# facebookresearch/dmc-net

Measured on AMD Instinct MI355X. Metric: clips/sec (3-seg 224x224) DMC-gen+ResNet-18 train step, higher is better.
Workload: dtype f32

## Files before the change

dmc-net_amd/_lib.py:

```python
import ctypes
import os

PKG = os.path.dirname(os.path.abspath(__file__))
LIB_PATH = os.environ.get("DMC_HIP_LIB", os.path.join(PKG, "libdmcnet_hip.so"))

_P = ctypes.c_void_p
_I = ctypes.c_int
_F = ctypes.c_float
_Z = ctypes.c_size_t
_L = ctypes.c_long

SIGNATURES = {
    "dmc_version": (_I, []),
    "dmc_last_error": (ctypes.c_char_p, []),
    "dmc_profile_mark": (_I, [_P]),
    "dmc_set_option": (_I, [ctypes.c_char_p, _I]),
    "dmc_get_option": (_I, [ctypes.c_char_p]),
    "dmc_gen_tiny_workspace_bytes": (_Z, []),
    "dmc_gen_tiny_saved_bytes": (_Z, [_I, _I, _I]),
    "dmc_gen_tiny_gbuf_bytes": (_Z, [_I, _I, _I]),
    "dmc_gen_tiny_partials_bytes": (_Z, [_I, _I, _I]),
    "dmc_gen_tiny_fwd": (_I, [_P, _P, _P, _P, _P, _P, _P, _I, _I, _I, _I, _P]),
    "dmc_gen_tiny_mse_partials_bytes": (_Z, []),
    "dmc_gen_tiny_fwd_mse": (_I, [_P] * 10 + [_I, _I, _I, _I, _P]),
# ... 29 lines not shown
    "dmc_conv_nhwc_stat_blocks": (_I, [_I] * 8),
    "dmc_conv_nhwc_fwd": (_I, [_P] * 7 + [_I] * 11 + [_P]),
    "dmc_conv_nhwc_stats_final": (_I, [_P, _I, _I, ctypes.c_long, _P, _P, _P, _F, _F, _P]),
    "dmc_conv_nhwc_wt_bytes": (_Z, [_I] * 4),
    "dmc_conv_nhwc_presplit_supported": (_I, [_I, _I]),
    "dmc_conv_nhwc_split": (_I, [_P, _P, _P, _I, _I, _I, _I, _P]),
    "dmc_conv_nhwc_dgrad": (_I, [_P] * 4 + [_I] * 9 + [_P]),
    "dmc_conv_nhwc_dgrad_add": (_I, [_P] * 5 + [_I] * 9 + [_P]),
    "dmc_conv_nhwc_wgrad_bytes": (_Z, [_I] * 9),
    "dmc_conv_nhwc_wgrad": (_I, [_P] * 4 + [_I] * 9 + [_P]),
    "dmc_x3s_slices_bytes": (_Z, [_L, _I]),
    "dmc_x3s_split": (_I, [_P, _P, _L, _I, _P]),
    "dmc_x3s_merge": (_I, [_P, _P, _L, _I, _P]),
    "dmc_x3s_wpack_bytes": (_Z, [_I, _I]),
    "dmc_x3s_pack_weights": (_I, [_P, _P, _P, _I, _I, _P]),
    "dmc_x3s_conv_supported": (_I, [_I] * 5),
    "dmc_x3s_conv_stat_blocks": (_I, [_I] * 4),
    "dmc_x3s_conv_fwd": (_I, [_P] * 4 + [_I] * 6 + [_P]),
    "dmc_x3s_conv_dgrad": (_I, [_P] * 4 + [_I] * 5 + [_P]),
    "dmc_x3s_conv_wgrad_supported": (_I, [_I] * 5),
    "dmc_x3s_conv_wgrad_bytes": (_Z, [_I] * 5),
    "dmc_x3s_conv_wgrad": (_I, [_P] * 4 + [_I] * 5 + [_P]),
    "dmc_x3s_conv_dgrad_s2_supported": (_I, [_I] * 5),
    "dmc_x3s_pack_weights_s2": (_I, [_P, _P, _I, _I, _P]),
    "dmc_x3s_conv_dgrad_s2": (_I, [_P] * 3 + [_I] * 5 + [_P]),
    "dmc_x3q_wpack_bytes": (_Z, [_I, _I]),
    "dmc_x3q_supported": (_I, [_I] * 5),
    "dmc_x3q_stat_blocks": (_I, [_I] * 4),
    "dmc_x3q_split": (_I, [_P, _P, _I, _I, _I, _I, _P]),
    "dmc_x3q_merge": (_I, [_P, _P, _I, _I, _I, _I, _P]),
# ... 107 lines not shown
```

dmc-net_amd/csrc/conv_x3s.hip:

```cpp
#include "dmc_common.h"
#include "x3s_common.h"
#include <type_traits>

using namespace dmc;
using namespace dmc::x3;

namespace {

__global__ __launch_bounds__(256) void x3s_split_kernel(const float* __restrict__ x, unsigned short* __restrict__ xs, long M, int C) {
    const int c8 = C >> 3;
    const long total = M * c8;
    const int nchunk = C >> 4;
    for (long o = (long)blockIdx.x * 256 + threadIdx.x; o < total; o += (long)gridDim.x * 256) {
        const long m = o / c8;
        const int g = (int)(o - m * c8);
        const float4 a = reinterpret_cast<const float4*>(x)[2 * o], b = reinterpret_cast<const float4*>(x)[2 * o + 1];
        const float v[8] = {a.x, a.y, a.z, a.w, b.x, b.y, b.z, b.w};
        x3s_store8(xs, v, (size_t)M, nchunk, (size_t)m, g);
    }
}

__global__ __launch_bounds__(256) void x3s_merge_kernel(const unsigned short* __restrict__ xs, float* __restrict__ x, long M, int C) {
    const long total = M * C;
    const size_t plane = (size_t)M * 16;
    const int nchunk = C >> 4;
    for (long o = (long)blockIdx.x * 256 + threadIdx.x; o < total; o += (long)gridDim.x * 256) {
        const long m = o / C;
        const int c = (int)(o - m * C);
        const size_t w = ((size_t)(c >> 4) * M + m) * 16 + (c & 15);
        const float a = __uint_as_float((unsigned)xs[w] << 16);
        const float b = __uint_as_float((unsigned)xs[(size_t)nchunk * plane + w] << 16);
        const float d = __uint_as_float((unsigned)xs[(size_t)2 * nchunk * plane + w] << 16);
        x[o] = (a + b) + d;
    }
}

__global__ __launch_bounds__(256) void x3s_pack_w_kernel(const float* __restrict__ w, unsigned short* __restrict__ wf,
                                                         unsigned short* __restrict__ wt, int Cout, int Cin, int mirror) {
    const bool transposed = blockIdx.y == 1;
    unsigned short* dst = transposed ? wt : wf;
    if (!dst) return;
    const int R = transposed ? Cin : Cout, K = transposed ? Cout : Cin;
    const int nchunk = K >> 4;
    const long total = (long)R * 9 * K;
    for (long i = (long)blockIdx.x * 256 + threadIdx.x; i < total; i += (long)gridDim.x * 256) {
        long t = i;
        const int kk = (int)(t & 15); t >>= 4;
        const int rl = (int)(t & 63); t >>= 6;
        const int tap = (int)(t % 9); t /= 9;
        const int ch = (int)(t % nchunk);
        const int rt = (int)(t / nchunk);
        const int r = rt * 64 + rl, k = ch * 16 + kk;
        const float v = transposed ? w[((long)k * 9 + (mirror ? 8 - tap : tap)) * Cin + r] : w[((long)r * 9 + tap) * Cin + k];
        unsigned u0, u1, u2;
        split3(v, u0, u1, u2);
        const size_t base = ((((size_t)(rt * nchunk + ch) * 9 + tap) * 3) * 64 + rl) * 16 + (kk ^ (((rl >> 3) & 1) << 3));
        dst[base] = (unsigned short)(u0 >> 16);
        dst[base + 64 * 16] = (unsigned short)(u1 >> 16);
        dst[base + 2 * 64 * 16] = (unsigned short)(u2 >> 16);
    }
}

struct X3Args {
    const void* xs;
    const void* wp;
    float* y;
    const float* addend;
    double* stat_part;
    int N, H, W, K, R;
    int M;
    unsigned plane_bytes;
    const float* bnb_y = nullptr;
    const float* bnb_stats = nullptr;
    const float* bnb_gamma = nullptr;
    const float* bnb_beta = nullptr;
    const unsigned char* bnb_mask = nullptr;
    int bnb_relu = 0;
    double* bnb_part = nullptr;
    int part_blocks = -1;
    int ablate;
};

template <int WM, int WN, int TM, int TN, int PPMAX, bool STAG = false, int CLS = 1>
__global__ __launch_bounds__(WM * WN * 64) void x3s_conv_kernel(X3Args a) {
    constexpr int NW = WM * WN, BM = 32 * TM * WM, BN = 32 * TN * WN;
    static_assert(BN == 64, "packed weight image is 64 rows wide");
    static_assert(PPMAX % 32 == 0 || PPMAX % 32 == 1, "patch transfers move 32 pixel rows");
    constexpr int PSL = PPMAX * 32;
    constexpr int PB = 3 * PSL;
    constexpr int WB = 3 * 3 * BN * 32;
    constexpr int WOFF = 2 * PB;
    static_assert(!STAG || NW >= 4, "two transfer groups need four waves");
    constexpr int NA = STAG ? NW / 2 : NW, NB = NW - (STAG ? NA : 0);
    constexpr int NDW = (PPMAX / 32 + NA - 1) / NA;
    constexpr int NEW = WB / 1024;
    constexpr int NEWW = (NEW + NB - 1) / NB;
    extern __shared__ __attribute__((aligned(1024))) char lds_x3[];

    const int tid = threadIdx.x, lane = tid & 63;
    const int wave = __builtin_amdgcn_readfirstlane(tid >> 6);
    const int wm = wave % WM, wn = wave / WM;
// ... 2 lines not shown

    const int HW = a.H * a.W, PW = a.W;
    constexpr int ZROW = PPMAX - 1;
    const int m0 = blockIdx.x * BM;
    const int mlast = (m0 + BM < a.M ? m0 + BM : a.M) - 1;
    const int r_first = m0 / PW, r_last = mlast / PW;
    const int f0 = (r_first > 0 ? r_first - 1 : 0) * PW;
    const int f1 = (r_last + 2) * PW < a.M ? (r_last + 2) * PW : a.M;
    const int PP = f1 - f0;
    const int ND = (PP + 31) >> 5;

    unsigned pvoff[NDW];
#pragma unroll
    for (int k = 0; k < NDW; ++k) {
        const int pr = 32 * (wave + NA * k) + (lane >> 1), h = lane & 1;
        pvoff[k] = pr < PP ? (unsigned)(f0 + pr) * 32u + (unsigned)((h ^ ((pr >> 3) & 1)) << 4) : OOB;
    }
    int xaddr[TM][9];
#pragma unroll
    for (int i = 0; i < TM; ++i) {
        int m = m0 + (wm * TM + i) * 32 + l31;
        if (m > mlast) m = mlast;
        const int n = m / HW, rem = m - n * HW, yy = rem / a.W, xx = rem - yy * a.W;
        const int pp = m - f0;
#pragma unroll
        for (int t = 0; t < 9; ++t) {
            const int dx = CLS == 4 ? (t % 3 == 0 ? 1 : 0) : t % 3 - 1, dy = CLS == 4 ? (t / 3 == 0 ? 1 : 0) : t / 3 - 1;
            const int row = (xx + dx >= 0 && xx + dx < a.W && yy + dy >= 0 && yy + dy < a.H) ? pp + dy * PW + dx : ZROW;
            xaddr[i][t] = row * 32 + ((khalf ^ ((row >> 3) & 1)) << 4);
        }
    }
    const int waddr = (wn * TN * 32 + l31) * 32 + ((khalf ^ ((l31 >> 3) & 1)) << 4);

    const u32x4 srd_x = make_srd(a.xs);
    const int nchunk = a.K >> 4, S = 3 * nchunk;
    const u32x4 srd_w = make_srd(reinterpret_cast<const char*>(a.wp) + (size_t)blockIdx.y * S * WB);
    const unsigned lane16 = (unsigned)lane * 16u;

    const bool grp_a = wave < NA, grp_b = !STAG || wave >= NA;
    const int wb = STAG ? wave - NA : wave;
    auto dma_weight = [&](int step, int wbuf, int k) {
        const int e = wb + NB * k;
        if (e < NEW) dma_buf16(srd_w, lane16, (unsigned)(step * WB + e * 1024), lds0 + WOFF + wbuf * WB + e * 1024);
    };
    auto dma_patch = [&](int chunk, int slice, int pbuf, int k) {
        const int d = wave + NA * k;
        if (d < ND) dma_buf16(srd_x, pvoff[k], (unsigned)(slice * nchunk + chunk) * a.plane_bytes, lds0 + pbuf * PB + slice * PSL + d * 1024);
// ... 103 lines not shown
                if (s + 2 < S) issue_weights(s + 2, wbuf);
                if (vc < nchunk) issue_patch(vc, q == 2 ? 0 : q + 1, q == 2 ? pbuf : (pbuf ^ 1));
            }
            if (s + 1 < S) load_frags(NP{}, NWB{}, NT{}, FB);
            mfma_frags(FA, T2{}, nothing);
        }
    };
    using I0 = std::integral_constant<int, 0>;
    using I1 = std::integral_constant<int, 1>;
    using Q0 = std::integral_constant<int, 0>;
    using Q1 = std::integral_constant<int, 1>;
    using Q2 = std::integral_constant<int, 2>;

    if (tid < 12)
        *reinterpret_cast<float4*>(lds_x3 + (tid >> 1) * PSL + ZROW * 32 + (tid & 1) * 16) = make_float4(0.f, 0.f, 0.f, 0.f);
    issue_weights(0, 0);
    issue_patch(0, 0, 0); issue_patch(0, 1, 0); issue_patch(0, 2, 0);
    asm volatile("s_waitcnt vmcnt(0)" ::: "memory");
    __builtin_amdgcn_s_barrier();
    if (dma_on) {
        if (!STAG && S > 1) issue_weights(1, 1);
        if (nchunk > 1) issue_patch(1, 0, 1);
    }
    Frag F0, F1;
    load_frags(I0{}, I0{}, Q0{}, F0);
#pragma unroll 1
    for (int c = 0; c < ((DMC_ABL(a.ablate) & 256) ? 0 : nchunk); c += 2) {
        step(I0{}, I0{}, Q0{}, F0, F1, c);
        step(I0{}, I1{}, Q1{}, F1, F0, c);
        step(I0{}, I0{}, Q2{}, F0, F1, c);
        step(I1{}, I1{}, Q0{}, F1, F0, c + 1);
        step(I1{}, I0{}, Q1{}, F0, F1, c + 1);
        step(I1{}, I1{}, Q2{}, F1, F0, c + 1);
    }

    static_assert(WN == 1 && TN == 2, "epilogue: a wave owns all 64 channels of its pixels");
    constexpr int EP = 272, ETILE = 32 * TM * EP;
    char* etile = lds_x3 + wave * ETILE;
    const int mw0 = m0 + wm * TM * 32;
    const int rbase = blockIdx.y * BN;
#pragma unroll
    for (int cl = 0; cl < CLS; ++cl) {
#pragma unroll
        for (int i = 0; i < TM; ++i) {
            const bool ok = mw0 + 32 * i + l31 <= mlast;
#pragma unroll
            for (int j = 0; j < TN; ++j)
#pragma unroll
                for (int g = 0; g < 4; ++g) {
                    float4 v = make_float4(acc[cl][i][j][4 * g], acc[cl][i][j][4 * g + 1], acc[cl][i][j][4 * g + 2], acc[cl][i][j][4 * g + 3]);
                    if (!ok) v = make_float4(0.f, 0.f, 0.f, 0.f);
                    *reinterpret_cast<float4*>(etile + (32 * i + l31) * EP + (32 * j + 8 * g + 4 * khalf) * 4) = v;
                }
        }
        if (!(DMC_ABL(a.ablate) & 128)) {
#pragma unroll
            for (int it = 0; it < 8 * TM; ++it) {
                const int prow = 4 * it + (lane >> 4);
                const int m = mw0 + prow;
// ... 86 lines not shown
    int worst = 0;
    long tiles = (M + BM - 1) / BM;
    if (tiles > W) tiles = W;
    for (long t = 0; t < tiles; ++t) {
        const long m0 = t * BM, ml = (m0 + BM < M ? m0 + BM : M) - 1;
        const long r0 = m0 / W, r1 = ml / W;
        const long f0 = (r0 > 0 ? r0 - 1 : 0) * W, f1 = (r1 + 2) * W;
        if ((int)(f1 - f0) + 1 > worst) worst = (int)(f1 - f0) + 1;
    }
    return worst;
}

struct X3Cfg { int id, BM, PPMAX, threads; };
constexpr X3Cfg X3CFGS[] = {{0, 256, 608, 512}, {1, 128, 320, 256}, {2, 64, 192, 128}, {3, 256, 608, 256}, {4, 128, 225, 256}};

bool x3s_shape_ok(int N, int H, int W, int K, int R) {
    if (N <= 0 || H <= 0 || W <= 0 || K % 32 != 0 || R % 64 != 0 || K <= 0 || R <= 0) return false;
    const long M = (long)N * H * W;
    return M * (K > R ? K : R) * 6 < (1L << 31);
}

int x3s_choose(int N, int H, int W, int R) {
    const long M = (long)N * H * W;
    const int forced = option(OPT_CONV_CFG);
    if (forced >= 101 && forced <= 105 && patch_pixels_max(N, H, W, X3CFGS[forced - 101].BM) <= X3CFGS[forced - 101].PPMAX) return forced - 101;
    if (forced != 106 && patch_pixels_max(N, H, W, X3CFGS[4].BM) <= X3CFGS[4].PPMAX && ((M + X3CFGS[4].BM - 1) / X3CFGS[4].BM) * (R / 64) >= 512)
        return 4;
    int fallback = -1;
    for (const X3Cfg& c : X3CFGS) {
        if (c.id > 2 || patch_pixels_max(N, H, W, c.BM) > c.PPMAX) continue;
        const long wgs = ((M + c.BM - 1) / c.BM) * (R / 64);
        if (wgs >= 160) return c.id;
        fallback = c.id;
    }
    return fallback;
}

template <int WM, int TM, int PPMAX>
int launch_x3s(const X3Args& a, hipStream_t s) {
    constexpr int BM = 32 * TM * WM;
    constexpr size_t op_bytes = 2 * 3 * PPMAX * 32 + 2 * 3 * 3 * 64 * 32, ep_bytes = 2 * (size_t)BM * 272 + 8192;
    constexpr size_t lds_bytes = op_bytes > ep_bytes ? op_bytes : ep_bytes;
    dim3 grid((a.M + BM - 1) / BM, a.R / 64);
    if ((a.stat_part || a.bnb_part) && a.part_blocks >= 0 && (unsigned)a.part_blocks != grid.x)
        return fail(DMC_E_INVALID, "x3s_conv: statistics partials have %d rows but this launch writes %u (dmc_x3s_conv_stat_blocks was "
                                   "called under another conv_cfg option?)", a.part_blocks, grid.x);
    if constexpr (WM >= 4) {
        if (!(option(OPT_CONV_ABLATE) & 512)) {
            static LdsLimit lim_attr2;
    const hipError_t attr2 = lim_attr2.raise(reinterpret_cast<const void*>(&x3s_conv_kernel<WM, 1, TM, 2, PPMAX, true>), (int)lds_bytes);
            if (attr2 != hipSuccess) return fail(DMC_E_LAUNCH, "x3s_conv: cannot raise the dynamic LDS limit: %s", hipGetErrorString(attr2));
            x3s_conv_kernel<WM, 1, TM, 2, PPMAX, true><<<grid, WM * 64, lds_bytes, s>>>(a);
            return check_launch("x3s_conv");
        }
    }
    static LdsLimit lim_attr;
    const hipError_t attr = lim_attr.raise(reinterpret_cast<const void*>(&x3s_conv_kernel<WM, 1, TM, 2, PPMAX>), (int)lds_bytes);
    if (attr != hipSuccess) return fail(DMC_E_LAUNCH, "x3s_conv: cannot raise the dynamic LDS limit: %s", hipGetErrorString(attr));
    x3s_conv_kernel<WM, 1, TM, 2, PPMAX><<<grid, WM * 64, lds_bytes, s>>>(a);
    return check_launch("x3s_conv");
}

struct X3Bnb { const float *y, *stats, *gamma, *beta; const unsigned char* mask; int relu; double* part; };

int run_x3s(const void* xs, const void* wp, const float* addend, float* y, double* stat_part, int part_blocks, int N, int H, int W,
            int K, int R, hipStream_t s, const X3Bnb* bnb = nullptr) {
    if (!xs || !wp || !y) return fail(DMC_E_INVALID, "x3s_conv: null pointer");
    if (!x3s_shape_ok(N, H, W, K, R)) return fail(DMC_E_INVALID, "x3s_conv: unsupported shape N=%d H=%d W=%d K=%d R=%d", N, H, W, K, R);
    const int cfg = x3s_choose(N, H, W, R);
    X3Args a;
    a.xs = xs; a.wp = wp; a.y = y; a.addend = addend; a.stat_part = stat_part;
    a.N = N; a.H = H; a.W = W; a.K = K; a.R = R; a.M = N * H * W;
    a.plane_bytes = (unsigned)a.M * 32u;
    a.part_blocks = part_blocks;
    if ((stat_part || bnb) && part_blocks <= 0) return fail(DMC_E_INVALID, "x3s_conv: stat_blocks must be the row count of the partials");
    if (bnb) {
        a.bnb_y = bnb->y; a.bnb_stats = bnb->stats; a.bnb_gamma = bnb->gamma; a.bnb_beta = bnb->beta; a.bnb_mask = bnb->mask;
        a.bnb_relu = bnb->relu; a.bnb_part = bnb->part;
    }
    a.ablate = option(OPT_CONV_ABLATE);
    if (DMC_ABL(a.ablate) & 32) a.stat_part = nullptr;
    switch (cfg) {
        case 0: return launch_x3s<8, 1, 608>(a, s);
        case 1: return launch_x3s<4, 1, 320>(a, s);
        case 2: return launch_x3s<2, 1, 192>(a, s);
        case 3: return launch_x3s<4, 2, 608>(a, s);
        case 4: return launch_x3s<4, 1, 225>(a, s);
        default: return fail(DMC_E_INVALID, "x3s_conv: the patch of a %d x %d image does not fit the LDS", H, W);
    }
}

struct X3WgArgs {
    const void* xs;
    const void* dys;
    float* part;
    int N, H, Cin, Cout;
    unsigned plane_bytes;
    int steps, per_group, tiles_ci;
};

template <int W_, int R>
struct WgGeom {
// ... 227 lines not shown

int dmc_x3s_split(const float* x, void* xs, long M, int C, dmc_stream_t stream) {
    if (!x || !xs || M <= 0 || C <= 0 || C % 16 != 0) return fail(DMC_E_INVALID, "dmc_x3s_split: bad argument");
    x3s_split_kernel<<<stream_blocks(M * (C / 8)), 256, 0, (hipStream_t)stream>>>(x, static_cast<unsigned short*>(xs), M, C);
    return check_launch("x3s_split");
}

int dmc_x3s_merge(const void* xs, float* x, long M, int C, dmc_stream_t stream) {
    if (!x || !xs || M <= 0 || C <= 0 || C % 16 != 0) return fail(DMC_E_INVALID, "dmc_x3s_merge: bad argument");
    x3s_merge_kernel<<<stream_blocks(M * C), 256, 0, (hipStream_t)stream>>>(static_cast<const unsigned short*>(xs), x, M, C);
    return check_launch("x3s_merge");
}

size_t dmc_x3s_wpack_bytes(int Cin, int Cout) { return (size_t)Cin * (size_t)Cout * 9 * 6; }

int dmc_x3s_pack_weights(const float* w, void* wpack_f, void* wpack_t, int Cin, int Cout, dmc_stream_t stream) {
    if (!w || (!wpack_f && !wpack_t) || Cin % 64 != 0 || Cout % 64 != 0 || Cin <= 0 || Cout <= 0)
        return fail(DMC_E_INVALID, "dmc_x3s_pack_weights: bad argument");
    const long total = (long)Cin * Cout * 9;
    x3s_pack_w_kernel<<<dim3(stream_blocks(total) > 1024 ? 1024 : stream_blocks(total), 2), 256, 0, (hipStream_t)stream>>>(
        w, static_cast<unsigned short*>(wpack_f), static_cast<unsigned short*>(wpack_t), Cout, Cin, 1);
    return check_launch("x3s_pack_w");
}

int dmc_x3s_conv_supported(int N, int H, int W, int Cin, int Cout) {
    return Cin % 64 == 0 && Cout % 64 == 0 && x3s_shape_ok(N, H, W, Cin, Cout) && x3s_shape_ok(N, H, W, Cout, Cin) &&
           x3s_choose(N, H, W, Cout) >= 0 && x3s_choose(N, H, W, Cin) >= 0 ? 1 : 0;
}

int dmc_x3s_conv_stat_blocks(int N, int H, int W, int Cout) {
    const int cfg = x3s_choose(N, H, W, Cout);
    if (cfg < 0) return 0;
    const long M = (long)N * H * W;
    return (int)((M + X3CFGS[cfg].BM - 1) / X3CFGS[cfg].BM);
}

// ... 37 lines not shown
        case 14: return launch_x3s_wgrad<14, 4>(p, a, dw, s);
        default: return launch_x3s_wgrad<7, 9>(p, a, dw, s);
    }
}

int dmc_x3s_conv_dgrad_s2_supported(int N, int OH, int OW, int Cin, int Cout) {
    return Cin % 64 == 0 && Cout % 64 == 0 && x3s_shape_ok(N, OH, OW, Cout, Cin) && (long)N * OH * OW * 4 * Cin * 4 < (1L << 40) &&
           patch_pixels_max(N, OH, OW, 128) <= 320 ? 1 : 0;
}

int dmc_x3s_pack_weights_s2(const float* w, void* wpack_t2, int Cin, int Cout, dmc_stream_t stream) {
    if (!w || !wpack_t2 || Cin % 64 != 0 || Cout % 64 != 0 || Cin <= 0 || Cout <= 0)
        return fail(DMC_E_INVALID, "dmc_x3s_pack_weights_s2: bad argument");
    const long total = (long)Cin * Cout * 9;
    x3s_pack_w_kernel<<<dim3(stream_blocks(total) > 1024 ? 1024 : stream_blocks(total), 2), 256, 0, (hipStream_t)stream>>>(
        w, nullptr, static_cast<unsigned short*>(wpack_t2), Cout, Cin, 0);
    return check_launch("x3s_pack_w_s2");
}

int dmc_x3s_conv_dgrad_s2(const void* dys, const void* wpack_t2, float* dx, int N, int OH, int OW, int Cin, int Cout,
                          dmc_stream_t stream) {
    if (!dys || !wpack_t2 || !dx) return fail(DMC_E_INVALID, "dmc_x3s_conv_dgrad_s2: null pointer");
    if (!dmc_x3s_conv_dgrad_s2_supported(N, OH, OW, Cin, Cout))
        return fail(DMC_E_INVALID, "dmc_x3s_conv_dgrad_s2: unsupported shape N=%d OH=%d OW=%d Cin=%d Cout=%d", N, OH, OW, Cin, Cout);
    X3Args a;
    a.xs = dys; a.wp = wpack_t2; a.y = dx; a.addend = nullptr; a.stat_part = nullptr;
    a.N = N; a.H = OH; a.W = OW; a.K = Cout; a.R = Cin; a.M = N * OH * OW;
    a.plane_bytes = (unsigned)a.M * 32u;
    a.ablate = option(OPT_CONV_ABLATE);
    constexpr size_t lds_bytes = 2 * 3 * 320 * 32 + 2 * 3 * 3 * 64 * 32;
    static LdsLimit lim_attr;
    const hipError_t attr = lim_attr.raise(reinterpret_cast<const void*>(&x3s_conv_kernel<4, 1, 1, 2, 320, true, 4>), (int)lds_bytes);
    if (attr != hipSuccess) return fail(DMC_E_LAUNCH, "x3s_conv_dgrad_s2: cannot raise the dynamic LDS limit: %s", hipGetErrorString(attr));
    dim3 grid((a.M + 127) / 128, Cin / 64);
    x3s_conv_kernel<4, 1, 1, 2, 320, true, 4><<<grid, 256, lds_bytes, (hipStream_t)stream>>>(a);
    return check_launch("x3s_conv_dgrad_s2");
}

int dmc_x3s_conv_dgrad_bnb(const void* dys, const void* wpack_t, const float* addend, float* dx, const float* bn_y,
// ... 14 lines not shown
```

dmc-net_amd/csrc/dmc_common.h:

```cpp
#pragma once
#include <hip/hip_runtime.h>
#include <stdarg.h>
#include <stdio.h>

#include <atomic>

#include "dmcnet_hip.h"

namespace dmc {

inline char* err_buf() {
    static thread_local char buf[512] = {0};
    return buf;
}
inline int fail(int code, const char* fmt, ...) {
    va_list ap;
    va_start(ap, fmt);
    vsnprintf(err_buf(), 512, fmt, ap);
    va_end(ap);
    return code;
}
inline int check_launch(const char* what) {
    hipError_t e = hipGetLastError();
    if (e != hipSuccess) return fail(DMC_E_LAUNCH, "%s: %s", what, hipGetErrorString(e));
// ... 2 lines not shown

struct LdsLimit {
    std::atomic<unsigned long long> raised{0};
    hipError_t raise(const void* kernel, int bytes) {
        int dev = 0;
        hipError_t e = hipGetDevice(&dev);
        if (e != hipSuccess) return e;
        if (dev >= 0 && dev < 64 && ((raised.load(std::memory_order_relaxed) >> dev) & 1ull)) return hipSuccess;
        e = hipFuncSetAttribute(kernel, hipFuncAttributeMaxDynamicSharedMemorySize, bytes);
        if (e == hipSuccess && dev >= 0 && dev < 64) raised.fetch_or(1ull << dev, std::memory_order_relaxed);
        return e;
    }
};

enum Option { OPT_GEN_LAYER_PATH = 0, OPT_GEN_GATHER, OPT_GEN_FUSE45, OPT_GEN_WGRAD_PATH, OPT_GEN_FUSE_FWD,
              OPT_GEN_FUSE_BWD, OPT_GEN_FRAMES, OPT_CONV_PATH, OPT_CONV_CFG, OPT_CONV_ABLATE, OPT_GEN_ABLATE, OPT_CONV_ARITH, OPT_CONV3D_WGRAD, OPT_GEN_X3, OPT_GEN_WINO, OPT_GEN_STAGGER, OPT_GEN_FUSED, OPT_GRID_RESERVE_CUS, OPT_COUNT };
int option(Option o);
inline int persistent_cus(int hw) {
    const int r = option(OPT_GRID_RESERVE_CUS);
    int n = hw - (r > 0 ? r : 0);
    n -= n % 8;
    return n < 8 ? (hw < 8 ? hw : 8) : n;
}
#ifdef DMC_MEASURE
#define DMC_ABL(x) (x)
constexpr bool MEASURE_BUILD = true;
#else
#define DMC_ABL(x) 0
constexpr bool MEASURE_BUILD = false;
#endif
constexpr bool measure_only(int o) { return o == OPT_GEN_ABLATE || o == OPT_CONV_ABLATE || o == OPT_GEN_STAGGER; }
// ... 130 lines not shown
```

dmc-net_amd/csrc/losses.hip:

```cpp
#include <atomic>
#include <string.h>

#include "dmc_common.h"

using namespace dmc;

namespace {

constexpr int MSE_BLOCKS = 2048;

__device__ __forceinline__ double wave_sum(double v) {
#pragma unroll
    for (int o = 32; o > 0; o >>= 1) v += __shfl_down(v, o, 64);
    return v;
}
__device__ __forceinline__ float wave_sum(float v) {
#pragma unroll
    for (int o = 32; o > 0; o >>= 1) v += __shfl_down(v, o, 64);
    return v;
}
__device__ __forceinline__ float wave_max(float v) {
#pragma unroll
    for (int o = 32; o > 0; o >>= 1) v = fmaxf(v, __shfl_down(v, o, 64));
    return v;
// ... 96 lines not shown
                const float g = t_ok ? (p - (c == t ? 1.f : 0.f)) * inv_n : NAN;
                for (int s = 0; s < S; ++s) grad[((size_t)b * S + s) * C + c] = g;
            }
        }
    }
    if (lane == 0) wave_loss[wave] = loss;
    __syncthreads();
    if (threadIdx.x == 0) {
        float s = 0.f;
        for (int w = 0; w < 16; ++w) s += wave_loss[w];
        *loss_out = s / (float)B;
    }
}

const char* const OPTION_NAMES[OPT_COUNT] = {"gen_layer_path", "gen_gather", "gen_fuse45", "gen_wgrad_path",
                                             "gen_fuse_fwd", "gen_fuse_bwd", "gen_frames", "conv_path", "conv_cfg", "conv_ablate", "gen_ablate", "conv_arith", "conv3d_wgrad", "gen_x3", "gen_wino", "gen_stagger", "gen_fused", "grid_reserve_cus"};
std::atomic<int> g_options[OPT_COUNT] = {{1}, {1}, {1}, {5}, {1}, {1}, {0}, {1}, {0}, {0}, {0}, {1}, {2}, {2}, {768}, {0}, {1}, {0}};
int option_index(const char* name) {
    if (!name) return -1;
    for (int i = 0; i < OPT_COUNT; ++i)
        if (strcmp(name, OPTION_NAMES[i]) == 0) return i;
    return -1;
}

}

namespace dmc {
int option(Option o) { return !MEASURE_BUILD && measure_only(o) ? 0 : g_options[o].load(std::memory_order_relaxed); }
}

__global__ void dmc_profile_mark_kernel() {}

// ... 68 lines not shown
```

dmc-net_amd/csrc/x3s_common.h:

```cpp
#pragma once
#include "dmc_common.h"

namespace dmc {
namespace x3 {

typedef float f32x16 __attribute__((ext_vector_type(16)));
typedef __bf16 bf16x8 __attribute__((ext_vector_type(8)));
typedef unsigned u32x4 __attribute__((ext_vector_type(4)));
typedef const __attribute__((address_space(3))) char* lds_cptr;

__device__ __forceinline__ f32x16 mfma_bf16(const u32x4& a, const u32x4& b, const f32x16& c) {
    return __builtin_amdgcn_mfma_f32_32x32x16_bf16(__builtin_bit_cast(bf16x8, a), __builtin_bit_cast(bf16x8, b), c, 0, 0, 0);
}

__device__ __forceinline__ void split3(float v, unsigned& u0, unsigned& u1, unsigned& u2) {
    u0 = __float_as_uint(v);
    const float r1 = v - __uint_as_float(u0 & 0xffff0000u);
    u1 = __float_as_uint(r1);
    u2 = __float_as_uint(r1 - __uint_as_float(u1 & 0xffff0000u));
}
__device__ __forceinline__ unsigned pack_hi(unsigned hi_of_second, unsigned hi_of_first) {
    return __builtin_amdgcn_perm(hi_of_second, hi_of_first, 0x07060302u);
}

// ... 45 lines not shown
__device__ __forceinline__ void wg_group_base(const WgGroupPos& p, int N, int W, unsigned img_bytes, unsigned& tbase, unsigned& img_off) {
    const bool in = p.n >= 0 && p.n < N;
    tbase = in ? (unsigned)((p.y - 1) * W) * 32u : NOPIX;
    img_off = in ? (unsigned)p.n * img_bytes : 0u;
}
__device__ __forceinline__ unsigned wg_lane_off(unsigned tbase, unsigned pre, unsigned img_bytes) {
    const unsigned t = tbase + pre;
    return t < img_bytes ? t : OOB;
}

typedef float f32x4 __attribute__((ext_vector_type(4)));
__device__ __forceinline__ f32x4 mfma16(const u32x4& a, const u32x4& b, const f32x4& c) {
    return __builtin_amdgcn_mfma_f32_16x16x32_bf16(__builtin_bit_cast(bf16x8, a), __builtin_bit_cast(bf16x8, b), c, 0, 0, 0);
}

__device__ __forceinline__ void split8(const float4& lo, const float4& hi, u32x4& s0, u32x4& s1, u32x4& s2) {
    const float v[8] = {lo.x, lo.y, lo.z, lo.w, hi.x, hi.y, hi.z, hi.w};
    unsigned u0[8], u1[8], u2[8];
#pragma unroll
    for (int e = 0; e < 8; ++e) split3(v[e], u0[e], u1[e], u2[e]);
#pragma unroll
    for (int e = 0; e < 4; ++e) {
        s0[e] = pack_hi(u0[2 * e + 1], u0[2 * e]);
        s1[e] = pack_hi(u1[2 * e + 1], u1[2 * e]);
        s2[e] = pack_hi(u2[2 * e + 1], u2[2 * e]);
    }
}

}
}
// ... 1 lines not shown
```

include/dmcnet_hip.h:

```cpp
#ifndef DMCNET_HIP_H
#define DMCNET_HIP_H

#include <stddef.h>
#include <stdint.h>

#ifdef __cplusplus
extern "C" {
#endif

#define DMC_OK 0
#define DMC_E_INVALID (-1)
#define DMC_E_LAUNCH (-2)

typedef void* dmc_stream_t;

int dmc_version(void);
const char* dmc_last_error(void);
int dmc_set_option(const char* name, int value);
int dmc_get_option(const char* name);
int dmc_profile_mark(dmc_stream_t stream);


size_t dmc_gen_tiny_workspace_bytes(void);
size_t dmc_gen_tiny_saved_bytes(int N, int H, int W);
// ... 94 lines not shown
size_t dmc_conv_nhwc_wt_bytes(int Cin, int Cout, int KH, int KW);
int dmc_conv_nhwc_presplit_supported(int Cin, int Cout);
int dmc_conv_nhwc_split(const float* w, void* wpack_f, void* wpack_t, int Cin, int Cout, int KH, int KW, dmc_stream_t stream);
int dmc_conv_nhwc_dgrad(const float* dy, const float* w, float* wt, float* dx, int N, int H, int W, int Cin,
                        int Cout, int KH, int KW, int stride, int pad, dmc_stream_t stream);
int dmc_conv_nhwc_dgrad_add(const float* dy, const float* w, float* wt, const float* addend, float* dx, int N, int H, int W,
                            int Cin, int Cout, int KH, int KW, int stride, int pad, dmc_stream_t stream);
size_t dmc_conv_nhwc_wgrad_bytes(int N, int H, int W, int Cin, int Cout, int KH, int KW, int stride, int pad);
int dmc_conv_nhwc_wgrad(const float* x, const float* dy, float* dw, float* workspace, int N, int H, int W,
                        int Cin, int Cout, int KH, int KW, int stride, int pad, dmc_stream_t stream);

size_t dmc_x3s_slices_bytes(long M, int C);
int dmc_x3s_split(const float* x, void* xs, long M, int C, dmc_stream_t stream);
int dmc_x3s_merge(const void* xs, float* x, long M, int C, dmc_stream_t stream);
size_t dmc_x3s_wpack_bytes(int Cin, int Cout);
int dmc_x3s_pack_weights(const float* w, void* wpack_f, void* wpack_t, int Cin, int Cout, dmc_stream_t stream);
int dmc_x3s_conv_supported(int N, int H, int W, int Cin, int Cout);
int dmc_x3s_conv_stat_blocks(int N, int H, int W, int Cout);
int dmc_x3s_conv_fwd(const void* xs, const void* wpack_f, float* y, double* stat_partials, int stat_blocks, int N, int H, int W,
                     int Cin, int Cout, dmc_stream_t stream);
int dmc_x3s_conv_dgrad(const void* dys, const void* wpack_t, const float* addend, float* dx, int N, int H, int W, int Cin,
                       int Cout, dmc_stream_t stream);
int dmc_x3s_conv_wgrad_supported(int N, int H, int W, int Cin, int Cout);
size_t dmc_x3s_conv_wgrad_bytes(int N, int H, int W, int Cin, int Cout);
int dmc_x3s_conv_wgrad(const void* xs, const void* dys, float* dw, float* workspace, int N, int H, int W, int Cin, int Cout,
                       dmc_stream_t stream);
int dmc_x3s_conv_dgrad_s2_supported(int N, int OH, int OW, int Cin, int Cout);
int dmc_x3s_pack_weights_s2(const float* w, void* wpack_t2, int Cin, int Cout, dmc_stream_t stream);
int dmc_x3s_conv_dgrad_s2(const void* dys, const void* wpack_t2, float* dx, int N, int OH, int OW, int Cin, int Cout,
                          dmc_stream_t stream);
// ... 151 lines not shown
```

Baseline: 3578.

## Add 16x16x32 MFMA inner loop and matching weight layout for x3s convolutions

Adds an alternative inner loop to the split-bf16 3x3 convolution kernel that uses 16x16x32 bf16 MFMA instead of 32x32x16. It regroups the K dimension into 9 groups of tap/chunk pairs per 32 channels, with a new packed weight layout, a three-buffer weight pipeline and a staged epilogue. By default it is enabled for 64x64 and 512x512 channel shapes. The aim is higher matrix-core throughput and fewer LDS loads per MFMA. In exchange it adds a host-side registry that checks the packed layout matches the loop chosen at launch, plus extra register pressure.

```diff
diff --git a/dmc-net_amd/_lib.py b/dmc-net_amd/_lib.py
--- a/dmc-net_amd/_lib.py
+++ b/dmc-net_amd/_lib.py
@@ -67,6 +67,9 @@
     "dmc_x3s_merge": (_I, [_P, _P, _L, _I, _P]),
     "dmc_x3s_wpack_bytes": (_Z, [_I, _I]),
     "dmc_x3s_pack_weights": (_I, [_P, _P, _P, _I, _I, _P]),
+    "dmc_x3s_conv_loop": (_I, [_I] * 3),
+    "dmc_x3s_kgroup_unit": (_I, [_I] * 2),
+    "dmc_x3s_wpack_indices": (_I, [_I] * 3 + [_P]),
     "dmc_x3s_conv_supported": (_I, [_I] * 5),
     "dmc_x3s_conv_stat_blocks": (_I, [_I] * 4),
     "dmc_x3s_conv_fwd": (_I, [_P] * 4 + [_I] * 6 + [_P]),
diff --git a/dmc-net_amd/csrc/conv_x3s.hip b/dmc-net_amd/csrc/conv_x3s.hip
--- a/dmc-net_amd/csrc/conv_x3s.hip
+++ b/dmc-net_amd/csrc/conv_x3s.hip
@@ -1,6 +1,8 @@
 #include "dmc_common.h"
 #include "x3s_common.h"
+#include <mutex>
 #include <type_traits>
+#include <unordered_map>
 
 using namespace dmc;
 using namespace dmc::x3;
@@ -36,10 +38,12 @@
 }
 
 __global__ __launch_bounds__(256) void x3s_pack_w_kernel(const float* __restrict__ w, unsigned short* __restrict__ wf,
-                                                         unsigned short* __restrict__ wt, int Cout, int Cin, int mirror) {
+                                                         unsigned short* __restrict__ wt, int Cout, int Cin, int mirror, int loop_f,
+                                                         int loop_t) {
     const bool transposed = blockIdx.y == 1;
     unsigned short* dst = transposed ? wt : wf;
     if (!dst) return;
+    const bool loop16 = (transposed ? loop_t : loop_f) != 0;
     const int R = transposed ? Cin : Cout, K = transposed ? Cout : Cin;
     const int nchunk = K >> 4;
     const long total = (long)R * 9 * K;
@@ -54,10 +58,15 @@
         const float v = transposed ? w[((long)k * 9 + (mirror ? 8 - tap : tap)) * Cin + r] : w[((long)r * 9 + tap) * Cin + k];
         unsigned u0, u1, u2;
         split3(v, u0, u1, u2);
-        const size_t base = ((((size_t)(rt * nchunk + ch) * 9 + tap) * 3) * 64 + rl) * 16 + (kk ^ (((rl >> 3) & 1) << 3));
-        dst[base] = (unsigned short)(u0 >> 16);
-        dst[base + 64 * 16] = (unsigned short)(u1 >> 16);
-        dst[base + 2 * 64 * 16] = (unsigned short)(u2 >> 16);
+        if (loop16) {
+            dst[x3s_w16_index(K, r, k, tap, 0)] = (unsigned short)(u0 >> 16);
+            dst[x3s_w16_index(K, r, k, tap, 1)] = (unsigned short)(u1 >> 16);
+            dst[x3s_w16_index(K, r, k, tap, 2)] = (unsigned short)(u2 >> 16);
+        } else {
+            dst[x3s_w32_index(K, r, k, tap, 0)] = (unsigned short)(u0 >> 16);
+            dst[x3s_w32_index(K, r, k, tap, 1)] = (unsigned short)(u1 >> 16);
+            dst[x3s_w32_index(K, r, k, tap, 2)] = (unsigned short)(u2 >> 16);
+        }
     }
 }
 
@@ -81,10 +90,11 @@
     int ablate;
 };
 
-template <int WM, int WN, int TM, int TN, int PPMAX, bool STAG = false, int CLS = 1>
+template <int WM, int WN, int TM, int TN, int PPMAX, bool STAG = false, int CLS = 1, int MF = 0>
 __global__ __launch_bounds__(WM * WN * 64) void x3s_conv_kernel(X3Args a) {
     constexpr int NW = WM * WN, BM = 32 * TM * WM, BN = 32 * TN * WN;
     static_assert(BN == 64, "packed weight image is 64 rows wide");
+    static_assert(!MF || (TM == 1 && CLS == 1), "the 16x16x32 loop is built for one 32-pixel tile per wave, stride 1");
     static_assert(PPMAX % 32 == 0 || PPMAX % 32 == 1, "patch transfers move 32 pixel rows");
     constexpr int PSL = PPMAX * 32;
     constexpr int PB = 3 * PSL;
@@ -117,7 +127,7 @@
 #pragma unroll
     for (int k = 0; k < NDW; ++k) {
         const int pr = 32 * (wave + NA * k) + (lane >> 1), h = lane & 1;
-        pvoff[k] = pr < PP ? (unsigned)(f0 + pr) * 32u + (unsigned)((h ^ ((pr >> 3) & 1)) << 4) : OOB;
+        pvoff[k] = pr < PP ? (unsigned)(f0 + pr) * 32u + (unsigned)((h ^ (MF ? 0 : (pr >> 3) & 1)) << 4) : OOB;
     }
     int xaddr[TM][9];
 #pragma unroll
@@ -134,6 +144,27 @@
         }
     }
     const int waddr = (wn * TN * 32 + l31) * 32 + ((khalf ^ ((l31 >> 3) & 1)) << 4);
+    const int l15 = lane & 15, sel = lane >> 5, h16 = ((lane >> 4) & 1) << 4;
+    int xg[2][X3S_G16];
+    if constexpr (MF) {
+#pragma unroll
+        for (int i = 0; i < 2; ++i) {
+            int m = m0 + wm * 32 + 16 * i + l15;
+            if (m > mlast) m = mlast;
+            const int n = m / HW, rem = m - n * HW, yy = rem / a.W, xx = rem - yy * a.W;
+            const int pp = m - f0;
+            int rowt[9];
+#pragma unroll
+            for (int t = 0; t < 9; ++t) {
+                const int dx = t % 3 - 1, dy = t / 3 - 1;
+                rowt[t] = (xx + dx >= 0 && xx + dx < a.W && yy + dy >= 0 && yy + dy < a.H) ? pp + dy * PW + dx : ZROW;
+            }
+#pragma unroll
+            for (int g = 0; g < X3S_G16; ++g)
+                xg[i][g] = (sel ? rowt[x3s_g16_tap(g, 1)] * 32 + x3s_g16_chunk(g, 1) * PB : rowt[x3s_g16_tap(g, 0)] * 32 + x3s_g16_chunk(g, 0) * PB) + h16;
+        }
+    }
+    const int waddr16 = sel * 512 + l15 * 32 + h16;
 
     const u32x4 srd_x = make_srd(a.xs);
     const int nchunk = a.K >> 4, S = 3 * nchunk;
@@ -267,24 +298,159 @@
 
     if (tid < 12)
         *reinterpret_cast<float4*>(lds_x3 + (tid >> 1) * PSL + ZROW * 32 + (tid & 1) * 16) = make_float4(0.f, 0.f, 0.f, 0.f);
-    issue_weights(0, 0);
-    issue_patch(0, 0, 0); issue_patch(0, 1, 0); issue_patch(0, 2, 0);
-    asm volatile("s_waitcnt vmcnt(0)" ::: "memory");
-    __builtin_amdgcn_s_barrier();
-    if (dma_on) {
-        if (!STAG && S > 1) issue_weights(1, 1);
-        if (nchunk > 1) issue_patch(1, 0, 1);
-    }
-    Frag F0, F1;
-    load_frags(I0{}, I0{}, Q0{}, F0);
+    if constexpr (MF) {
+        constexpr int WG = 3 * BN * 64;
+        static_assert(3 * WG == 2 * WB, "three group buffers take the place of the two tap-row buffers");
+        constexpr int NEW16 = WG / 1024, NEWW16 = (NEW16 + NB - 1) / NB;
+        const int NG = (nchunk >> 1) * X3S_G16;
+        auto dma_weight16 = [&](int G, int wbuf, int k) {
+            const int e = wb + NB * k;
+            if (e < NEW16) dma_buf16(srd_w, lane16, (unsigned)(G * WG + e * 1024), lds0 + WOFF + wbuf * WG + e * 1024);
+        };
+        f32x4 acc16[2][4];
+#pragma unroll
+        for (int i = 0; i < 2; ++i)
+#pragma unroll
+            for (int j = 0; j < 4; ++j)
+#pragma unroll
+                for (int e = 0; e < 4; ++e) acc16[i][j][e] = 0.f;
+        struct Frag16 { u32x4 X[2][3], W[4][3]; };
+        auto load_frag16 = [&](auto gic, auto wbufc, auto qc, Frag16& f) {
+            constexpr int gi = decltype(gic)::value, wbuf = decltype(wbufc)::value, q = decltype(qc)::value, sl = q / 6, o = q % 6;
+            if constexpr (o < 4)
+                f.W[o][sl] = *reinterpret_cast<const __attribute__((address_space(3))) u32x4*>(L + waddr16 + (WOFF + wbuf * WG + (sl * 4 + o) * 1024));
+            else
+                f.X[o - 4][sl] = *reinterpret_cast<const __attribute__((address_space(3))) u32x4*>(L + xg[o - 4][gi] + sl * PSL);
+        };
+        auto group16 = [&](auto gic, Frag16& FA, Frag16& FB, int c) {
+            constexpr int gi = decltype(gic)::value;
+            using GN = std::integral_constant<int, (gi + 1) % X3S_G16>;
+            using WN_ = std::integral_constant<int, (gi + 1) % 3>;
+            constexpr int wfill = (gi + 2) % 3;
+            constexpr int pslice = gi == 0 ? 1 : gi == 1 ? 2 : gi == 4 ? 0 : gi == 5 ? 1 : gi == 6 ? 2 : gi == 8 ? 0 : -1;
+            constexpr int pdc = gi <= 1 ? 1 : gi == 8 ? 3 : 2, pbuf = gi >= 4 && gi <= 6 ? 0 : 1;
+            const int G = (c >> 1) * X3S_G16 + gi;
+            if (DMC_ABL(a.ablate) & 16) asm volatile("s_waitcnt lgkmcnt(0)" ::: "memory");
+            else asm volatile("s_waitcnt vmcnt(0) lgkmcnt(0)" ::: "memory");
+            __builtin_amdgcn_s_barrier();
+            const bool gow = grp_b && dma_on && G + 2 < NG;
+            const bool gop = pslice >= 0 && grp_a && dma_on && c + pdc < nchunk;
+            if constexpr (!STAG) {
+                if (gow) {
+#pragma unroll
+                    for (int k = 0; k < NEWW16; ++k) dma_weight16(G + 2, wfill, k);
+                }
+                if (gop) {
+#pragma unroll
+                    for (int k = 0; k < NDW; ++k) dma_patch(c + pdc, pslice < 0 ? 0 : pslice, pbuf, k);
+                }
+            }
+            auto product = [&](auto pc) {
+                constexpr int p = decltype(pc)::value;
+                constexpr int WS[6] = {0, 0, 0, 1, 1, 2}, XS[6] = {2, 1, 0, 1, 0, 0};
+                load_frag16(GN{}, WN_{}, std::integral_constant<int, 3 * p>{}, FB);
+                load_frag16(GN{}, WN_{}, std::integral_constant<int, 3 * p + 1>{}, FB);
+                load_frag16(GN{}, WN_{}, std::integral_constant<int, 3 * p + 2>{}, FB);
+#pragma unroll
+                for (int i = 0; i < 2; ++i)
+#pragma unroll
+                    for (int j = 0; j < 4; ++j) acc16[i][j] = mfma16(FA.W[j][WS[p]], FA.X[i][XS[p]], acc16[i][j]);
+#pragma unroll
+                for (int k = 0; k < 3; ++k) {
+                    __builtin_amdgcn_sched_group_barrier(0x008, 1, 0);
+                    __builtin_amdgcn_sched_group_barrier(0x100, 1, 0);
+                }
+                __builtin_amdgcn_sched_group_barrier(0x008, 5, 0);
+                if constexpr (STAG) {
+                    if (gow) {
+#pragma unroll
+                        for (int k = p; k < NEWW16; k += 6) dma_weight16(G + 2, wfill, k);
+                    }
+                    if (gop) {
+#pragma unroll
+                        for (int k = p; k < NDW; k += 6) dma_patch(c + pdc, pslice < 0 ? 0 : pslice, pbuf, k);
+                    }
+                }
+            };
+            product(std::integral_constant<int, 0>{}); product(std::integral_constant<int, 1>{});
+            product(std::integral_constant<int, 2>{}); product(std::integral_constant<int, 3>{});
+            product(std::integral_constant<int, 4>{}); product(std::integral_constant<int, 5>{});
+        };
+        auto pair16 = [&](Frag16& FA, Frag16& FB, int c) {
+            group16(std::integral_constant<int, 0>{}, FA, FB, c); group16(std::integral_constant<int, 1>{}, FB, FA, c);
+            group16(std::integral_constant<int, 2>{}, FA, FB, c); group16(std::integral_constant<int, 3>{}, FB, FA, c);
+            group16(std::integral_constant<int, 4>{}, FA, FB, c); group16(std::integral_constant<int, 5>{}, FB, FA, c);
+            group16(std::integral_constant<int, 6>{}, FA, FB, c); group16(std::integral_constant<int, 7>{}, FB, FA, c);
+            group16(std::integral_constant<int, 8>{}, FA, FB, c);
+        };
+        if (grp_b) {
+#pragma unroll
+            for (int k = 0; k < NEWW16; ++k) dma_weight16(0, 0, k);
+        }
+        issue_patch(0, 0, 0); issue_patch(0, 1, 0); issue_patch(0, 2, 0);
+        asm volatile("s_waitcnt vmcnt(0)" ::: "memory");
+        __builtin_amdgcn_s_barrier();
+        if (dma_on) {
+            if (grp_b && NG > 1) {
+#pragma unroll
+                for (int k = 0; k < NEWW16; ++k) dma_weight16(1, 1, k);
+            }
+            if (nchunk > 1) issue_patch(1, 0, 1);
+        }
+        Frag16 F0, F1;
+        {
+            using Z = std::integral_constant<int, 0>;
+            load_frag16(Z{}, Z{}, std::integral_constant<int, 0>{}, F0); load_frag16(Z{}, Z{}, std::integral_constant<int, 1>{}, F0);
+            load_frag16(Z{}, Z{}, std::integral_constant<int, 2>{}, F0); load_frag16(Z{}, Z{}, std::integral_constant<int, 3>{}, F0);
+            load_frag16(Z{}, Z{}, std::integral_constant<int, 4>{}, F0); load_frag16(Z{}, Z{}, std::integral_constant<int, 5>{}, F0);
+            load_frag16(Z{}, Z{}, std::integral_constant<int, 6>{}, F0); load_frag16(Z{}, Z{}, std::integral_constant<int, 7>{}, F0);
+            load_frag16(Z{}, Z{}, std::integral_constant<int, 8>{}, F0); load_frag16(Z{}, Z{}, std::integral_constant<int, 9>{}, F0);
+            load_frag16(Z{}, Z{}, std::integral_constant<int, 10>{}, F0); load_frag16(Z{}, Z{}, std::integral_constant<int, 11>{}, F0);
+            load_frag16(Z{}, Z{}, std::integral_constant<int, 12>{}, F0); load_frag16(Z{}, Z{}, std::integral_constant<int, 13>{}, F0);
+            load_frag16(Z{}, Z{}, std::integral_constant<int, 14>{}, F0); load_frag16(Z{}, Z{}, std::integral_constant<int, 15>{}, F0);
+            load_frag16(Z{}, Z{}, std::integral_constant<int, 16>{}, F0); load_frag16(Z{}, Z{}, std::integral_constant<int, 17>{}, F0);
+        }
+        const int nrun = (DMC_ABL(a.ablate) & 256) ? 0 : nchunk;
+        int c = 0;
 #pragma unroll 1
-    for (int c = 0; c < ((DMC_ABL(a.ablate) & 256) ? 0 : nchunk); c += 2) {
-        step(I0{}, I0{}, Q0{}, F0, F1, c);
-        step(I0{}, I1{}, Q1{}, F1, F0, c);
-        step(I0{}, I0{}, Q2{}, F0, F1, c);
-        step(I1{}, I1{}, Q0{}, F1, F0, c + 1);
-        step(I1{}, I0{}, Q1{}, F0, F1, c + 1);
-        step(I1{}, I1{}, Q2{}, F1, F0, c + 1);
+        for (; c + 4 <= nrun; c += 4) {
+            pair16(F0, F1, c);
+            pair16(F1, F0, c + 2);
+        }
+        if (c < nrun) pair16(F0, F1, c);
+        {
+            char* et = lds_x3 + wave * (32 * 272);
+#pragma unroll
+            for (int i = 0; i < 2; ++i) {
+                const bool ok = m0 + wm * 32 + 16 * i + l15 <= mlast;
+#pragma unroll
+                for (int j = 0; j < 4; ++j) {
+                    float4 v = make_float4(acc16[i][j][0], acc16[i][j][1], acc16[i][j][2], acc16[i][j][3]);
+                    if (!ok) v = make_float4(0.f, 0.f, 0.f, 0.f);
+                    *reinterpret_cast<float4*>(et + (16 * i + l15) * 272 + (16 * j + 4 * (lane >> 4)) * 4) = v;
+                }
+            }
+        }
+    } else {
+        issue_weights(0, 0);
+        issue_patch(0, 0, 0); issue_patch(0, 1, 0); issue_patch(0, 2, 0);
+        asm volatile("s_waitcnt vmcnt(0)" ::: "memory");
+        __builtin_amdgcn_s_barrier();
+        if (dma_on) {
+            if (!STAG && S > 1) issue_weights(1, 1);
+            if (nchunk > 1) issue_patch(1, 0, 1);
+        }
+        Frag F0, F1;
+        load_frags(I0{}, I0{}, Q0{}, F0);
+    #pragma unroll 1
+        for (int c = 0; c < ((DMC_ABL(a.ablate) & 256) ? 0 : nchunk); c += 2) {
+            step(I0{}, I0{}, Q0{}, F0, F1, c);
+            step(I0{}, I1{}, Q1{}, F1, F0, c);
+            step(I0{}, I0{}, Q2{}, F0, F1, c);
+            step(I1{}, I1{}, Q0{}, F1, F0, c + 1);
+            step(I1{}, I0{}, Q1{}, F0, F1, c + 1);
+            step(I1{}, I1{}, Q2{}, F1, F0, c + 1);
+        }
     }
 
     static_assert(WN == 1 && TN == 2, "epilogue: a wave owns all 64 channels of its pixels");
@@ -295,7 +461,7 @@
 #pragma unroll
     for (int cl = 0; cl < CLS; ++cl) {
 #pragma unroll
-        for (int i = 0; i < TM; ++i) {
+        for (int i = 0; i < (MF ? 0 : TM); ++i) {
             const bool ok = mw0 + 32 * i + l31 <= mlast;
 #pragma unroll
             for (int j = 0; j < TN; ++j)
@@ -412,6 +578,30 @@
 struct X3Cfg { int id, BM, PPMAX, threads; };
 constexpr X3Cfg X3CFGS[] = {{0, 256, 608, 512}, {1, 128, 320, 256}, {2, 64, 192, 128}, {3, 256, 608, 256}, {4, 128, 225, 256}};
 
+bool x3s_loop16(int K, int R) {
+    const int o = option(OPT_CONV_MFMA);
+    if (o == 0) return false;
+    if (o == 1) return true;
+    return (K == 64 && R == 64) || (K == 512 && R == 512);
+}
+
+std::mutex g_wpack_mu;
+std::unordered_map<const void*, int> g_wpack_loop;
+void wpack_note(const void* p, int loop) {
+    if (!p) return;
+    std::lock_guard<std::mutex> lk(g_wpack_mu);
+    g_wpack_loop[p] = loop;
+}
+int wpack_check(const void* p, int loop, const char* who) {
+    std::lock_guard<std::mutex> lk(g_wpack_mu);
+    const auto it = g_wpack_loop.find(p);
+    if (it != g_wpack_loop.end() && it->second != loop)
+        return fail(DMC_E_INVALID, "%s: the weights were packed for the %s matrix loop but this launch runs the %s one (option conv_mfma "
+                                   "changed between dmc_x3s_pack_weights and the convolution?)", who, it->second ? "16x16x32" : "32x32x16",
+                    loop ? "16x16x32" : "32x32x16");
+    return DMC_OK;
+}
+
 bool x3s_shape_ok(int N, int H, int W, int K, int R) {
     if (N <= 0 || H <= 0 || W <= 0 || K % 32 != 0 || R % 64 != 0 || K <= 0 || R <= 0) return false;
     const long M = (long)N * H * W;
@@ -435,7 +625,7 @@
 }
 
 template <int WM, int TM, int PPMAX>
-int launch_x3s(const X3Args& a, hipStream_t s) {
+int launch_x3s(const X3Args& a, hipStream_t s, bool loop16) {
     constexpr int BM = 32 * TM * WM;
     constexpr size_t op_bytes = 2 * 3 * PPMAX * 32 + 2 * 3 * 3 * 64 * 32, ep_bytes = 2 * (size_t)BM * 272 + 8192;
     constexpr size_t lds_bytes = op_bytes > ep_bytes ? op_bytes : ep_bytes;
@@ -443,6 +633,18 @@
     if ((a.stat_part || a.bnb_part) && a.part_blocks >= 0 && (unsigned)a.part_blocks != grid.x)
         return fail(DMC_E_INVALID, "x3s_conv: statistics partials have %d rows but this launch writes %u (dmc_x3s_conv_stat_blocks was "
                                    "called under another conv_cfg option?)", a.part_blocks, grid.x);
+    if constexpr (TM == 1) {
+        if (loop16) {
+            constexpr bool ST = WM >= 4;
+            static LdsLimit lim_attr3;
+            const hipError_t attr3 = lim_attr3.raise(reinterpret_cast<const void*>(&x3s_conv_kernel<WM, 1, TM, 2, PPMAX, ST, 1, 1>), (int)lds_bytes);
+            if (attr3 != hipSuccess) return fail(DMC_E_LAUNCH, "x3s_conv: cannot raise the dynamic LDS limit: %s", hipGetErrorString(attr3));
+            x3s_conv_kernel<WM, 1, TM, 2, PPMAX, ST, 1, 1><<<grid, WM * 64, lds_bytes, s>>>(a);
+            return check_launch("x3s_conv");
+        }
+    } else if (loop16) {
+        return fail(DMC_E_INVALID, "x3s_conv: this tile configuration is built on the 32x32x16 loop only (option conv_mfma = 0)");
+    }
     if constexpr (WM >= 4) {
         if (!(option(OPT_CONV_ABLATE) & 512)) {
             static LdsLimit lim_attr2;
@@ -466,6 +668,8 @@
     if (!xs || !wp || !y) return fail(DMC_E_INVALID, "x3s_conv: null pointer");
     if (!x3s_shape_ok(N, H, W, K, R)) return fail(DMC_E_INVALID, "x3s_conv: unsupported shape N=%d H=%d W=%d K=%d R=%d", N, H, W, K, R);
     const int cfg = x3s_choose(N, H, W, R);
+    const bool loop16 = x3s_loop16(K, R);
+    if (int rc = wpack_check(wp, loop16 ? 1 : 0, "x3s_conv")) return rc;
     X3Args a;
     a.xs = xs; a.wp = wp; a.y = y; a.addend = addend; a.stat_part = stat_part;
     a.N = N; a.H = H; a.W = W; a.K = K; a.R = R; a.M = N * H * W;
@@ -479,11 +683,11 @@
     a.ablate = option(OPT_CONV_ABLATE);
     if (DMC_ABL(a.ablate) & 32) a.stat_part = nullptr;
     switch (cfg) {
-        case 0: return launch_x3s<8, 1, 608>(a, s);
-        case 1: return launch_x3s<4, 1, 320>(a, s);
-        case 2: return launch_x3s<2, 1, 192>(a, s);
-        case 3: return launch_x3s<4, 2, 608>(a, s);
-        case 4: return launch_x3s<4, 1, 225>(a, s);
+        case 0: return launch_x3s<8, 1, 608>(a, s, loop16);
+        case 1: return launch_x3s<4, 1, 320>(a, s, loop16);
+        case 2: return launch_x3s<2, 1, 192>(a, s, loop16);
+        case 3: return launch_x3s<4, 2, 608>(a, s, loop16);
+        case 4: return launch_x3s<4, 1, 225>(a, s, loop16);
         default: return fail(DMC_E_INVALID, "x3s_conv: the patch of a %d x %d image does not fit the LDS", H, W);
     }
 }
@@ -741,12 +945,36 @@
 
 size_t dmc_x3s_wpack_bytes(int Cin, int Cout) { return (size_t)Cin * (size_t)Cout * 9 * 6; }
 
+int dmc_x3s_conv_loop(int Cin, int Cout, int transposed) {
+    if (Cin <= 0 || Cout <= 0 || Cin % 64 != 0 || Cout % 64 != 0) return -1;
+    return (transposed ? x3s_loop16(Cout, Cin) : x3s_loop16(Cin, Cout)) ? 1 : 0;
+}
+
+int dmc_x3s_kgroup_unit(int group, int sel) {
+    if (group < 0 || group >= X3S_G16 || sel < 0 || sel > 1) return -1;
+    return x3s_g16_chunk(group, sel) * 9 + x3s_g16_tap(group, sel);
+}
+
+int dmc_x3s_wpack_indices(int loop, int R, int K, int* out) {
+    if (!out || (loop != 0 && loop != 1) || R <= 0 || K <= 0 || R % 64 != 0 || K % 32 != 0 || (long)R * K * 27 >= (1L << 31))
+        return fail(DMC_E_INVALID, "dmc_x3s_wpack_indices: bad argument");
+    size_t o = 0;
+    for (int r = 0; r < R; ++r)
+        for (int tap = 0; tap < 9; ++tap)
+            for (int k = 0; k < K; ++k)
+                for (int sl = 0; sl < 3; ++sl) out[o++] = (int)(loop ? x3s_w16_index(K, r, k, tap, sl) : x3s_w32_index(K, r, k, tap, sl));
+    return DMC_OK;
+}
+
 int dmc_x3s_pack_weights(const float* w, void* wpack_f, void* wpack_t, int Cin, int Cout, dmc_stream_t stream) {
     if (!w || (!wpack_f && !wpack_t) || Cin % 64 != 0 || Cout % 64 != 0 || Cin <= 0 || Cout <= 0)
         return fail(DMC_E_INVALID, "dmc_x3s_pack_weights: bad argument");
     const long total = (long)Cin * Cout * 9;
+    const int loop_f = x3s_loop16(Cin, Cout) ? 1 : 0, loop_t = x3s_loop16(Cout, Cin) ? 1 : 0;
     x3s_pack_w_kernel<<<dim3(stream_blocks(total) > 1024 ? 1024 : stream_blocks(total), 2), 256, 0, (hipStream_t)stream>>>(
-        w, static_cast<unsigned short*>(wpack_f), static_cast<unsigned short*>(wpack_t), Cout, Cin, 1);
+        w, static_cast<unsigned short*>(wpack_f), static_cast<unsigned short*>(wpack_t), Cout, Cin, 1, loop_f, loop_t);
+    wpack_note(wpack_f, loop_f);
+    wpack_note(wpack_t, loop_t);
     return check_launch("x3s_pack_w");
 }
 
@@ -814,7 +1042,8 @@
         return fail(DMC_E_INVALID, "dmc_x3s_pack_weights_s2: bad argument");
     const long total = (long)Cin * Cout * 9;
     x3s_pack_w_kernel<<<dim3(stream_blocks(total) > 1024 ? 1024 : stream_blocks(total), 2), 256, 0, (hipStream_t)stream>>>(
-        w, nullptr, static_cast<unsigned short*>(wpack_t2), Cout, Cin, 0);
+        w, nullptr, static_cast<unsigned short*>(wpack_t2), Cout, Cin, 0, 0, 0);
+    wpack_note(wpack_t2, 0);
     return check_launch("x3s_pack_w_s2");
 }
 
@@ -823,6 +1052,7 @@
     if (!dys || !wpack_t2 || !dx) return fail(DMC_E_INVALID, "dmc_x3s_conv_dgrad_s2: null pointer");
     if (!dmc_x3s_conv_dgrad_s2_supported(N, OH, OW, Cin, Cout))
         return fail(DMC_E_INVALID, "dmc_x3s_conv_dgrad_s2: unsupported shape N=%d OH=%d OW=%d Cin=%d Cout=%d", N, OH, OW, Cin, Cout);
+    if (int rc = wpack_check(wpack_t2, 0, "dmc_x3s_conv_dgrad_s2")) return rc;
     X3Args a;
     a.xs = dys; a.wp = wpack_t2; a.y = dx; a.addend = nullptr; a.stat_part = nullptr;
     a.N = N; a.H = OH; a.W = OW; a.K = Cout; a.R = Cin; a.M = N * OH * OW;
diff --git a/dmc-net_amd/csrc/dmc_common.h b/dmc-net_amd/csrc/dmc_common.h
--- a/dmc-net_amd/csrc/dmc_common.h
+++ b/dmc-net_amd/csrc/dmc_common.h
@@ -40,7 +40,7 @@
 };
 
 enum Option { OPT_GEN_LAYER_PATH = 0, OPT_GEN_GATHER, OPT_GEN_FUSE45, OPT_GEN_WGRAD_PATH, OPT_GEN_FUSE_FWD,
-              OPT_GEN_FUSE_BWD, OPT_GEN_FRAMES, OPT_CONV_PATH, OPT_CONV_CFG, OPT_CONV_ABLATE, OPT_GEN_ABLATE, OPT_CONV_ARITH, OPT_CONV3D_WGRAD, OPT_GEN_X3, OPT_GEN_WINO, OPT_GEN_STAGGER, OPT_GEN_FUSED, OPT_GRID_RESERVE_CUS, OPT_COUNT };
+              OPT_GEN_FUSE_BWD, OPT_GEN_FRAMES, OPT_CONV_PATH, OPT_CONV_CFG, OPT_CONV_ABLATE, OPT_GEN_ABLATE, OPT_CONV_ARITH, OPT_CONV3D_WGRAD, OPT_GEN_X3, OPT_GEN_WINO, OPT_GEN_STAGGER, OPT_GEN_FUSED, OPT_GRID_RESERVE_CUS, OPT_CONV_MFMA, OPT_COUNT };
 int option(Option o);
 inline int persistent_cus(int hw) {
     const int r = option(OPT_GRID_RESERVE_CUS);
diff --git a/dmc-net_amd/csrc/losses.hip b/dmc-net_amd/csrc/losses.hip
--- a/dmc-net_amd/csrc/losses.hip
+++ b/dmc-net_amd/csrc/losses.hip
@@ -134,8 +134,8 @@
 }
 
 const char* const OPTION_NAMES[OPT_COUNT] = {"gen_layer_path", "gen_gather", "gen_fuse45", "gen_wgrad_path",
-                                             "gen_fuse_fwd", "gen_fuse_bwd", "gen_frames", "conv_path", "conv_cfg", "conv_ablate", "gen_ablate", "conv_arith", "conv3d_wgrad", "gen_x3", "gen_wino", "gen_stagger", "gen_fused", "grid_reserve_cus"};
-std::atomic<int> g_options[OPT_COUNT] = {{1}, {1}, {1}, {5}, {1}, {1}, {0}, {1}, {0}, {0}, {0}, {1}, {2}, {2}, {768}, {0}, {1}, {0}};
+                                             "gen_fuse_fwd", "gen_fuse_bwd", "gen_frames", "conv_path", "conv_cfg", "conv_ablate", "gen_ablate", "conv_arith", "conv3d_wgrad", "gen_x3", "gen_wino", "gen_stagger", "gen_fused", "grid_reserve_cus", "conv_mfma"};
+std::atomic<int> g_options[OPT_COUNT] = {{1}, {1}, {1}, {5}, {1}, {1}, {0}, {1}, {0}, {0}, {0}, {1}, {2}, {2}, {768}, {0}, {1}, {0}, {2}};
 int option_index(const char* name) {
     if (!name) return -1;
     for (int i = 0; i < OPT_COUNT; ++i)
diff --git a/dmc-net_amd/csrc/x3s_common.h b/dmc-net_amd/csrc/x3s_common.h
--- a/dmc-net_amd/csrc/x3s_common.h
+++ b/dmc-net_amd/csrc/x3s_common.h
@@ -83,6 +83,19 @@
     return __builtin_amdgcn_mfma_f32_16x16x32_bf16(__builtin_bit_cast(bf16x8, a), __builtin_bit_cast(bf16x8, b), c, 0, 0, 0);
 }
 
+constexpr int X3S_G16 = 9;
+__host__ __device__ constexpr int x3s_g16_chunk(int group, int sel) { return (2 * group + sel) / 9; }
+__host__ __device__ constexpr int x3s_g16_tap(int group, int sel) { return (2 * group + sel) % 9; }
+__host__ __device__ inline size_t x3s_w32_index(int K, int r, int k, int tap, int slice) {
+    const int rl = r & 63, kk = k & 15;
+    return (((((size_t)(r >> 6) * (K >> 4) + (k >> 4)) * 9 + tap) * 3 + slice) * 64 + rl) * 16 + (kk ^ (((rl >> 3) & 1) << 3));
+}
+__host__ __device__ inline size_t x3s_w16_index(int K, int r, int k, int tap, int slice) {
+    const int rl = r & 63, ch = k >> 4, u = (ch & 1) * 9 + tap;
+    return ((((((size_t)(r >> 6) * (K >> 5) + (ch >> 1)) * X3S_G16 + (u >> 1)) * 3 + slice) * 4 + (rl >> 4)) * 2 + (u & 1)) * 256 +
+           (rl & 15) * 16 + (k & 15);
+}
+
 __device__ __forceinline__ void split8(const float4& lo, const float4& hi, u32x4& s0, u32x4& s1, u32x4& s2) {
     const float v[8] = {lo.x, lo.y, lo.z, lo.w, hi.x, hi.y, hi.z, hi.w};
     unsigned u0[8], u1[8], u2[8];
diff --git a/include/dmcnet_hip.h b/include/dmcnet_hip.h
--- a/include/dmcnet_hip.h
+++ b/include/dmcnet_hip.h
@@ -132,6 +132,9 @@
 int dmc_x3s_split(const float* x, void* xs, long M, int C, dmc_stream_t stream);
 int dmc_x3s_merge(const void* xs, float* x, long M, int C, dmc_stream_t stream);
 size_t dmc_x3s_wpack_bytes(int Cin, int Cout);
+int dmc_x3s_conv_loop(int Cin, int Cout, int transposed);
+int dmc_x3s_kgroup_unit(int group, int sel);
+int dmc_x3s_wpack_indices(int loop, int R, int K, int* out);
 int dmc_x3s_pack_weights(const float* w, void* wpack_f, void* wpack_t, int Cin, int Cout, dmc_stream_t stream);
 int dmc_x3s_conv_supported(int N, int H, int W, int Cin, int Cout);
 int dmc_x3s_conv_stat_blocks(int N, int H, int W, int Cout);
```

Result: no change. 3609 (median of 6 runs) (+0.9%).
